# bentotten/radiation_ppo

Hardware: AMD Instinct MI355X
Metric: env steps/sec (whole node) at 4096 envs; PPO iters/sec at 1/2/4/8 GPUs (higher is better)
Workload: dtype f32 policy / f64+int32 env

## Files before the change

include/radsearch.h:

```cpp
#ifndef RADSEARCH_H
#define RADSEARCH_H

#include <stddef.h>
#include <stdint.h>

#ifdef __cplusplus
extern "C" {
#endif

#define RS_ABI_VERSION 4
#define RS_OBS_DIM 11
#define RS_NUM_ACTIONS 9
#define RS_MAX_AGENTS 8
#define RS_MAX_OBS 7

typedef void* rs_stream_t;
typedef struct rs_handle rs_handle;

enum {
    RS_OK = 0,
    RS_ERR_INVALID_ARG = 1,
    RS_ERR_HIP = 2,
    RS_ERR_WORKSPACE = 3,
    RS_ERR_UNSUPPORTED = 4
};

enum {
    RS_ENVERR_ZERO_DIST = 1,
    RS_ENVERR_IDLE_STALL = 2,
    RS_ENVERR_CORRECT_CAP = 4,
    RS_ENVERR_BAD_ACTION = 8,
    RS_ENVERR_NO_PATH = 16
};

typedef struct rs_config {
    int32_t num_envs;
    int32_t num_agents;
    int32_t obstruction_count;
    int32_t enforce_grid_boundaries;
    int32_t bbox[4];
    int32_t observation_area[2];
    int32_t falloff;
    int32_t geom_group_size;
    uint32_t seed;
    uint32_t env_id_base;
    int32_t coord_noise;
    int32_t debug_spawn;
} rs_config;

typedef struct rs_info {
    uint8_t* out_of_bounds;
    int32_t* out_of_bounds_count;
    uint8_t* blocked;
    uint8_t* collision;
} rs_info;

const char* rs_strerror(int code);
int rs_abi_version(void);

size_t rs_state_bytes(const rs_config* cfg);

int rs_create(const rs_config* cfg, void* workspace, size_t workspace_bytes, rs_stream_t stream, rs_handle** out);
void rs_destroy(rs_handle* h);

int rs_state_field(rs_handle* h, const char* name, void** dev_ptr, int32_t* elem_bytes, int32_t* rows, int32_t* cols);

int rs_set_epoch_end(rs_handle* h, rs_stream_t stream);

int rs_reset(rs_handle* h, const uint8_t* mask, float* obs, float* reward, float* team, uint8_t* done,
             const rs_info* info, rs_stream_t stream);

int rs_refresh(rs_handle* h, const uint8_t* mask, const int32_t* src_xy, const int32_t* det_xy, const int32_t* intensity,
               const int32_t* bkg, const int32_t* num_obs, const int32_t* rects, float* obs, float* reward, float* team,
               uint8_t* done, const rs_info* info, rs_stream_t stream);

int rs_step(rs_handle* h, const int8_t* actions, float* obs, float* reward, float* team, uint8_t* done,
            const rs_info* info, rs_stream_t stream);

int rs_action_uniforms(rs_handle* h, float* u, rs_stream_t stream);

int rs_error_flags(rs_handle* h, rs_stream_t stream, uint32_t* flags_out);

int rs_gae(const float* rew, const float* val, const uint8_t* cut, const float* last_val, float* adv, float* ret,
           int32_t T, int32_t M, double gamma, double lam, rs_stream_t stream);

typedef struct rs_mlp_params {
    const float *w1, *b1, *w2, *b2, *w3, *b3;
} rs_mlp_params;

int rs_policy_forward(const rs_mlp_params* actor, const rs_mlp_params* critic, const float* x, int32_t M,
                      float* logits, float* value, rs_stream_t stream);

typedef struct rs_rollout_args {
    int32_t steps_per_epoch;
    int32_t steps_per_episode;
    float* obs;
    int64_t* act;
    float* logp;
    float* val;
    float* rew;
    float* last_val;
    uint8_t* cut;
    float* source_tar;
    float* cur_obs;
    double* w_count;
    double* w_mean;
    double* w_sq;
    double* w_std;
    int32_t* steps_in_ep;
    float* ep_ret;
    int32_t* done_count;
    int32_t* oob_count;
    double* ep_ret_sum;
    double* ep_len_sum;
    int32_t* ep_count;
    double* ep_ret_sq_sum;
    float* ep_ret_max;
    float* ep_ret_min;
} rs_rollout_args;

int rs_rollout(rs_handle* h, const rs_mlp_params* actor, const rs_mlp_params* critic, const rs_rollout_args* args,
               rs_stream_t stream);

typedef struct rs_ppo_batch {
    const float* x;
    const int64_t* act;
    const float* adv;
    const float* ret;
    const float* logp_old;
    const float* w;
    int32_t M;
    float clip_ratio, alpha, vf_coef;
} rs_ppo_batch;

size_t rs_ppo_grad_workspace_bytes(void);
#define RS_PPO_STATS_TAIL 16
#define RS_PPO_GRAD_FLOATS (10441 + RS_PPO_STATS_TAIL)
int rs_ppo_grad(const rs_mlp_params* actor, const rs_mlp_params* critic, const rs_ppo_batch* batch, float* grads,
                double* stats, void* workspace, const int32_t* stop_flag, rs_stream_t stream);

typedef struct rs_update_state {
    int32_t adam_step;
    int32_t stopped;
    int32_t iters;
    int32_t pad;
    double last_stats[5];
} rs_update_state;

int rs_adam_step(const rs_mlp_params* actor, const rs_mlp_params* critic, const float* grads, float* m, float* v,
                 const double* stats, rs_update_state* state, float lr, float kl_threshold, rs_stream_t stream);

int rs_ppo_update_step(const rs_mlp_params* actor, const rs_mlp_params* critic, const rs_ppo_batch* batch, float* grads,
                       double* stats, void* workspace, float* m, float* v, rs_update_state* state, float lr, float kl_threshold,
                       rs_stream_t stream);

typedef struct rs_maps rs_maps;
size_t rs_maps_state_bytes(int32_t num_envs, int32_t num_agents, int32_t steps_per_episode, int32_t map_x, int32_t map_y);
int rs_maps_create(int32_t num_envs, int32_t num_agents, int32_t steps_per_episode, int32_t map_x, int32_t map_y,
                   double resolution_accuracy, const float* visit_table, void* workspace, size_t workspace_bytes,
                   rs_stream_t stream, rs_maps** out);
void rs_maps_destroy(rs_maps* m);
int rs_maps_reset(rs_maps* m, const uint8_t* mask, rs_stream_t stream);
int rs_maps_update(rs_maps* m, rs_handle* env, const float* obs, const float* pred, const uint8_t* mask, rs_stream_t stream);
int rs_maps_stack(rs_maps* m, float* actor_stack, float* critic_stack, rs_stream_t stream);
int rs_maps_field(rs_maps* m, const char* name, void** dev_ptr, int32_t* elem_bytes, int32_t* rows, int32_t* cols);

int32_t rs_cnn_trunk_slab_row(int32_t in_channels);
int32_t rs_cnn_trunk_slab_rows(int64_t num_samples, int32_t in_channels);
int32_t rs_cnn_trunk_scratch_floats(int32_t in_channels);
int rs_cnn_trunk_forward(const float* maps, const int64_t* cells, const int64_t* pcells, int32_t num_agents, int32_t agent,
                         int64_t num_samples, const float* w1, const float* b1, const float* w2, const float* b2, float* a2,
                         float* p1, uint8_t* amax, uint16_t* relu_mask, float* wscratch, rs_stream_t stream);
int rs_cnn_trunk_backward(const float* maps, const int64_t* cells, const int64_t* pcells, int32_t num_agents, int32_t agent,
                          int64_t num_samples, const float* w2, const float* da2, const uint16_t* relu_mask, const float* p1,
                          const uint8_t* amax, float* slab, float* wscratch, rs_stream_t stream);

#define RS_PFGRU_PARTICLES 40
#define RS_PFGRU_HIDDEN 24
#define RS_PFGRU_WEIGHT_FLOATS 3472
int rs_pfgru_step(const float* weights, const float* obs, float* h, float* p, const int64_t* base_key, const int64_t* episode,
                  const int64_t* calls, const uint8_t* mask, int32_t carry_hidden, double alpha, float* pred, int32_t num_envs,
                  int32_t num_agents, rs_stream_t stream);
int rs_pfgru_pass(const float* weights, const float* obs, float* h, float* p, const int64_t* base_key, const int64_t* episode,
                  const int64_t* calls, double alpha, float* pred, const int32_t* alive, int32_t steps, int32_t episodes, rs_stream_t stream);
int rs_pfgru_step_recorded(const float* weights, const float* obs, float* h, float* p, const float* eps, const int32_t* idx,
                           const uint8_t* mask, int32_t carry_hidden, double alpha, float* pred, int32_t num_envs, int32_t num_agents,
                           rs_stream_t stream);
int rs_pfgru_reset(float* h, float* p, const int64_t* base_key, const int64_t* episode, const int64_t* calls, const uint8_t* mask,
                   int32_t num_envs, int32_t num_agents, rs_stream_t stream);

int32_t rs_pfgru_sized_weight_floats(int32_t hidden);
int rs_pfgru_sized_step(const float* weights, const float* obs, float* h, float* p, const int64_t* base_key, const int64_t* episode,
                        const int64_t* calls, const uint8_t* mask, int32_t carry_hidden, double alpha, float* pred, int32_t num_envs,
                        int32_t num_agents, int32_t hidden, rs_stream_t stream);
int rs_pfgru_sized_pass(const float* weights, const float* obs, float* h, float* p, const int64_t* base_key, const int64_t* episode,
                        const int64_t* calls, double alpha, float* pred, const int32_t* alive, int32_t steps, int32_t episodes, int32_t hidden,
                        rs_stream_t stream);
int rs_pfgru_sized_step_recorded(const float* weights, const float* obs, float* h, float* p, const float* eps, const int32_t* idx,
                                 const uint8_t* mask, int32_t carry_hidden, double alpha, float* pred, int32_t num_envs, int32_t num_agents,
                                 int32_t hidden, rs_stream_t stream);
int rs_pfgru_sized_reset(float* h, float* p, const int64_t* base_key, const int64_t* episode, const int64_t* calls, const uint8_t* mask,
                         int32_t num_envs, int32_t num_agents, int32_t hidden, rs_stream_t stream);

int rs_pfgru_draws(const int64_t* keys, int32_t episodes, int32_t steps, float* h0, float* eps, double* u, rs_stream_t stream);

#define RS_PFGRU_TRAIN_WEIGHT_FLOATS 3680
#define RS_PFGRU_TRAIN_GRAD_FLOATS 3376
int rs_pfgru_train(const float* weights, const float* obs, const float* target, const float* bp, const int64_t* lens, const float* w_ep,
                   const float* h0, const float* eps, const double* u, float* hs, float* ps, float* gates, int32_t* idx, float* loss,
                   float* grads, int32_t steps, int32_t episodes, double alpha, double l2_weight, double l1_weight, double elbo_weight,
                   rs_stream_t stream);
int rs_pfgru_train_keyed(const float* weights, const float* obs, const float* target, const float* bp, const int64_t* lens, const float* w_ep,
                         const int64_t* keys, float* h0, float* hs, float* ps, float* gates, int32_t* idx, float* loss, float* grads, int32_t steps,
                         int32_t episodes, double alpha, double l2_weight, double l1_weight, double elbo_weight, rs_stream_t stream);

int32_t rs_pfgru_sized_train_weight_floats(int32_t hidden);
int32_t rs_pfgru_sized_train_grad_floats(int32_t hidden);
int rs_pfgru_sized_draws(const int64_t* keys, int32_t episodes, int32_t steps, int32_t hidden, float* h0, float* eps, double* u,
                         rs_stream_t stream);
int rs_pfgru_sized_train(const float* weights, const float* obs, const float* target, const float* bp, const int64_t* lens, const float* w_ep,
                         const float* h0, const float* eps, const double* u, float* hs, float* ps, float* gates, int32_t* idx, float* loss,
                         float* grads, int32_t steps, int32_t episodes, double alpha, double l2_weight, double l1_weight, double elbo_weight,
                         int32_t hidden, rs_stream_t stream);

#define RS_GRU_HIDDEN 24
int rs_gru_forward(const float* gi, const float* h0, const float* whh_t, const float* bhh, float* hs, float* gates, int32_t steps,
                   int32_t episodes, rs_stream_t stream);
int rs_gru_backward(const float* dhs, const float* hs, const float* gates, const float* h0, const float* whh, float* dgi, float* dgh,
                    int32_t steps, int32_t episodes, rs_stream_t stream);

#define RS_RNN_POLICY_WEIGHT_FLOATS 5296
int rs_rnn_policy_step(const float* weights, const float* x, const float* loc, const float* h, const float* u, float* h_out,
                       float* logits, float* value, int64_t* act, float* logp, int32_t num_envs, rs_stream_t stream);
int rs_rnn_policy_step_rows(const float* weights, const float* x, int32_t x_stride, const float* loc, int32_t loc_stride, const float* h,
                            const float* u, int32_t u_stride, float* h_out, float* value, int64_t* act, float* logp, int8_t* act8,
                            int32_t act8_stride, const uint8_t* mask, int32_t num_envs, rs_stream_t stream);

int rs_a2c_heads_loss(const float* weights, const float* hs, const int64_t* act, const float* adv, const float* ret, const float* logp_old,
                      const float* sample_weight, float* dhs, float* dfac, float* tfac, float* stats, int64_t samples, double clip_ratio,
                      double vf_coef, rs_stream_t stream);

int32_t rs_rnn_sized_weight_floats(int32_t hid, int32_t pol, int32_t val);
int32_t rs_gru_sized_weight_floats(int32_t hid);
int32_t rs_gru_sized_gate_floats(int32_t hid);
int rs_rnn_sized_step(const float* weights, int32_t hid, int32_t pol, int32_t val, const float* x, int32_t x_stride, const float* loc,
                      int32_t loc_stride, const float* h, const float* u, int32_t u_stride, float* h_out, float* logits, float* value,
                      int64_t* act, float* logp, int8_t* act8, int32_t act8_stride, const uint8_t* mask, int32_t num_envs, rs_stream_t stream);
int rs_gru_sized_forward(const float* gi, const float* h0, const float* weights, float* hs, float* gates, int32_t hid, int32_t steps,
                         int32_t episodes, rs_stream_t stream);
int rs_gru_sized_backward(const float* dhs, const float* hs, const float* gates, const float* h0, const float* weights, float* dgi, float* dgh,
                          int32_t hid, int32_t steps, int32_t episodes, rs_stream_t stream);
int rs_a2c_sized_heads_loss(const float* weights, int32_t hid, int32_t pol, int32_t val, const float* hs, const int64_t* act, const float* adv,
                            const float* ret, const float* logp_old, const float* sample_weight, float* dhs, float* dfac, float* tfac,
                            float* stats, int64_t samples, double clip_ratio, double vf_coef, rs_stream_t stream);
int rs_gru_h0_reset_sized(float* h, const int64_t* base_key, const int64_t* episodes_begun, const uint8_t* mask, double scale, int32_t hid,
                          int32_t num_envs, int32_t num_agents, rs_stream_t stream);

int rs_cnn_trunk_prepare(int32_t in_channels, const float* w1, const float* b1, const float* w2, const float* b2, float* wscratch,
                         rs_stream_t stream);
int rs_cnn_trunk_infer(const float* maps, const int64_t* cells, const int64_t* pcells, int32_t num_agents, int32_t agent, int64_t num_samples,
                       const float* wscratch, float* a2, rs_stream_t stream);

int32_t rs_cnn_sized_slab_row(int32_t in_channels);
int32_t rs_cnn_sized_slab_rows(int64_t num_samples, int32_t map_side, int32_t in_channels);
int rs_cnn_sized_forward(const float* maps, const int64_t* cells, const int64_t* pcells, int32_t num_agents, int32_t agent,
                         int64_t num_samples, int32_t map_side, const float* w1, const float* b1, const float* w2, const float* b2,
                         float* a2, float* p1, uint8_t* amax, uint16_t* relu_mask, rs_stream_t stream);
int rs_cnn_sized_infer(const float* maps, const int64_t* cells, const int64_t* pcells, int32_t num_agents, int32_t agent, int64_t num_samples,
                       int32_t map_side, const float* w1, const float* b1, const float* w2, const float* b2, float* a2, rs_stream_t stream);
int rs_cnn_sized_backward(const float* maps, const int64_t* cells, const int64_t* pcells, int32_t num_agents, int32_t agent,
                          int64_t num_samples, int32_t map_side, const float* w2, const float* da2, const uint16_t* relu_mask,
                          const float* p1, const uint8_t* amax, float* slab, int32_t slab_rows, rs_stream_t stream);

int rs_cnn_head(const float* y1, const float* w2, const float* b2, const float* w3, const float* b3, int32_t out_dim, const float* u,
                int32_t u_stride, int64_t* act, float* logp, int8_t* act8, int32_t act8_stride, float* value, int32_t value_copies,
                int64_t value_stride, const uint8_t* mask, int32_t num_envs, rs_stream_t stream);

int rs_actor_loss(const float* logits, const int64_t* act, const float* adv, const float* logp_old, const float* sample_weight,
                  float* dlogits, float* stats, int64_t samples, double clip_ratio, rs_stream_t stream);

int rs_gru_h0_reset(float* h, const int64_t* base_key, const int64_t* episodes_begun, const uint8_t* mask, double scale, int32_t num_envs,
                    int32_t num_agents, rs_stream_t stream);

int rs_welford_update(double* count, double* mean, double* sq, double* std, const float* reading, int64_t stride, const uint8_t* mask,
                      int32_t num_envs, int32_t num_agents, rs_stream_t stream);
int rs_welford_reset(double* count, double* mean, double* sq, double* std, const uint8_t* mask, int32_t num_envs, int32_t num_agents,
                     rs_stream_t stream);
int rs_welford_standardize(const double* mean, const double* std, const float* reading, int64_t stride, float* out, int64_t out_stride,
                           int32_t streams, rs_stream_t stream);

int rs_epoch_stats(const uint8_t* out_of_bounds, const uint8_t* done, const float* ep_ret, const int32_t* steps_in_ep, const uint8_t* over,
                   double* acc_oob, double* acc_done, double* ep_cnt, double* ep_len, double* ret_sum, double* ret_sq, double* ret_max,
                   double* ret_min, int32_t num_envs, int32_t num_agents, rs_stream_t stream);

int rs_store_rows(const int64_t* t, const int64_t* act, const float* logp_val_boot, const float* x, const int32_t* src_x, const int32_t* src_y,
                  const float* rew, const uint8_t* cut, const uint8_t* boot, int64_t* buf_act, float* buf_logp, float* buf_val,
                  float* buf_last_val, float* buf_obs, float* buf_source, float* buf_rew, uint8_t* buf_cut, int32_t num_envs,
                  int32_t num_agents, int32_t steps_per_epoch, rs_stream_t stream);

typedef struct {
    int32_t num_envs, num_agents, steps_per_episode, team_reward;
    const float* env_obs;
    const float* env_reward;
    const float* env_team;
    const uint8_t* env_done;
    float* obs;
    float* ep_ret;
    int32_t* steps_in_ep;
    double* w_count; double* w_mean; double* w_sq; double* w_std;
    float* x;
    float* xb;
    float* reward_used;
    uint8_t* over; uint8_t* cut; uint8_t* boot;
    int64_t* pf_episode; int64_t* pf_calls; int64_t* episodes_begun;
    int64_t* t;
    const uint8_t* env_oob;
    const int32_t* env_src_x; const int32_t* env_src_y;
    uint8_t* done_copy; uint8_t* oob_copy;
    int32_t* src_copy;
    int64_t* complete_len;
} rs_collect_state;
int rs_collect_pre(const rs_collect_state* c, rs_stream_t stream);
int rs_collect_post_step(const rs_collect_state* c, int32_t epoch_ended, rs_stream_t stream);
int rs_collect_post_reset(const rs_collect_state* c, int32_t reset_hidden, rs_stream_t stream);

#ifdef __cplusplus
}
#endif
#endif
```

radiation_ppo_amd/_lib.py:

```python
import ctypes as C
import os

import torch

_PKG = os.path.dirname(os.path.abspath(__file__))
LIB_PATH = os.environ.get("RS_LIB_PATH") or os.path.join(_PKG, "lib", "librs_hip.so")

RS_OBS_DIM = 11
RS_MAX_AGENTS = 8
RS_MAX_OBS = 7

ENVERR_ZERO_DIST = 1
ENVERR_IDLE_STALL = 2
ENVERR_CORRECT_CAP = 4
ENVERR_BAD_ACTION = 8
ENVERR_NO_PATH = 16


class RsConfig(C.Structure):
    _fields_ = [
        ("num_envs", C.c_int32), ("num_agents", C.c_int32), ("obstruction_count", C.c_int32),
        ("enforce_grid_boundaries", C.c_int32), ("bbox", C.c_int32 * 4), ("observation_area", C.c_int32 * 2),
        ("falloff", C.c_int32), ("geom_group_size", C.c_int32), ("seed", C.c_uint32), ("env_id_base", C.c_uint32),
        ("coord_noise", C.c_int32), ("debug_spawn", C.c_int32),
    ]


class RsCollectState(C.Structure):
    _fields_ = [("num_envs", C.c_int32), ("num_agents", C.c_int32), ("steps_per_episode", C.c_int32), ("team_reward", C.c_int32)] + [
        (n, C.c_void_p) for n in ("env_obs", "env_reward", "env_team", "env_done", "obs", "ep_ret", "steps_in_ep", "w_count", "w_mean", "w_sq",
                                  "w_std", "x", "xb", "reward_used", "over", "cut", "boot", "pf_episode", "pf_calls", "episodes_begun", "t",
                                  "env_oob", "env_src_x", "env_src_y", "done_copy", "oob_copy", "src_copy", "complete_len")]


class RsMlpParams(C.Structure):
    _fields_ = [(n, C.c_void_p) for n in ("w1", "b1", "w2", "b2", "w3", "b3")]


class RsRolloutArgs(C.Structure):
    _fields_ = [("steps_per_epoch", C.c_int32), ("steps_per_episode", C.c_int32)] + [
        (n, C.c_void_p) for n in ("obs", "act", "logp", "val", "rew", "last_val", "cut", "source_tar", "cur_obs", "w_count",
                                  "w_mean", "w_sq", "w_std", "steps_in_ep", "ep_ret", "done_count", "oob_count",
                                  "ep_ret_sum", "ep_len_sum", "ep_count", "ep_ret_sq_sum", "ep_ret_max", "ep_ret_min")]


class RsPpoBatch(C.Structure):
    _fields_ = [("x", C.c_void_p), ("act", C.c_void_p), ("adv", C.c_void_p), ("ret", C.c_void_p), ("logp_old", C.c_void_p),
                ("w", C.c_void_p), ("M", C.c_int32), ("clip_ratio", C.c_float), ("alpha", C.c_float), ("vf_coef", C.c_float)]


class RsInfo(C.Structure):
    _fields_ = [("out_of_bounds", C.c_void_p), ("out_of_bounds_count", C.c_void_p), ("blocked", C.c_void_p),
                ("collision", C.c_void_p)]


SYMBOLS = [
    ("rs_strerror", C.c_char_p, [C.c_int]),
    ("rs_abi_version", C.c_int, []),
    ("rs_state_bytes", C.c_size_t, [C.POINTER(RsConfig)]),
    ("rs_create", C.c_int, [C.POINTER(RsConfig), C.c_void_p, C.c_size_t, C.c_void_p, C.POINTER(C.c_void_p)]),
    ("rs_destroy", None, [C.c_void_p]),
    ("rs_state_field", C.c_int, [C.c_void_p, C.c_char_p, C.POINTER(C.c_void_p), C.POINTER(C.c_int32),
                                 C.POINTER(C.c_int32), C.POINTER(C.c_int32)]),
    ("rs_set_epoch_end", C.c_int, [C.c_void_p, C.c_void_p]),
    ("rs_reset", C.c_int, [C.c_void_p, C.c_void_p, C.c_void_p, C.c_void_p, C.c_void_p, C.c_void_p,
                           C.POINTER(RsInfo), C.c_void_p]),
    ("rs_refresh", C.c_int, [C.c_void_p, C.c_void_p, C.c_void_p, C.c_void_p, C.c_void_p, C.c_void_p, C.c_void_p, C.c_void_p,
                             C.c_void_p, C.c_void_p, C.c_void_p, C.c_void_p, C.POINTER(RsInfo), C.c_void_p]),
    ("rs_step", C.c_int, [C.c_void_p, C.c_void_p, C.c_void_p, C.c_void_p, C.c_void_p, C.c_void_p,
                          C.POINTER(RsInfo), C.c_void_p]),
    ("rs_action_uniforms", C.c_int, [C.c_void_p, C.c_void_p, C.c_void_p]),
    ("rs_error_flags", C.c_int, [C.c_void_p, C.c_void_p, C.POINTER(C.c_uint32)]),
    ("rs_policy_forward", C.c_int, [C.POINTER(RsMlpParams), C.POINTER(RsMlpParams), C.c_void_p, C.c_int32, C.c_void_p,
                                    C.c_void_p, C.c_void_p]),
    ("rs_rollout", C.c_int, [C.c_void_p, C.POINTER(RsMlpParams), C.POINTER(RsMlpParams), C.POINTER(RsRolloutArgs), C.c_void_p]),
    ("rs_ppo_grad_workspace_bytes", C.c_size_t, []),
    ("rs_ppo_grad", C.c_int, [C.POINTER(RsMlpParams), C.POINTER(RsMlpParams), C.POINTER(RsPpoBatch), C.c_void_p, C.c_void_p,
                              C.c_void_p, C.c_void_p, C.c_void_p]),
    ("rs_adam_step", C.c_int, [C.POINTER(RsMlpParams), C.POINTER(RsMlpParams), C.c_void_p, C.c_void_p, C.c_void_p, C.c_void_p,
                               C.c_void_p, C.c_float, C.c_float, C.c_void_p]),
    ("rs_ppo_update_step", C.c_int, [C.POINTER(RsMlpParams), C.POINTER(RsMlpParams), C.POINTER(RsPpoBatch), C.c_void_p, C.c_void_p,
                                     C.c_void_p, C.c_void_p, C.c_void_p, C.c_void_p, C.c_float, C.c_float, C.c_void_p]),
    ("rs_maps_state_bytes", C.c_size_t, [C.c_int32, C.c_int32, C.c_int32, C.c_int32, C.c_int32]),
    ("rs_maps_create", C.c_int, [C.c_int32, C.c_int32, C.c_int32, C.c_int32, C.c_int32, C.c_double, C.c_void_p, C.c_void_p,
                                 C.c_size_t, C.c_void_p, C.POINTER(C.c_void_p)]),
    ("rs_maps_destroy", None, [C.c_void_p]),
    ("rs_maps_reset", C.c_int, [C.c_void_p, C.c_void_p, C.c_void_p]),
    ("rs_maps_update", C.c_int, [C.c_void_p, C.c_void_p, C.c_void_p, C.c_void_p, C.c_void_p, C.c_void_p]),
    ("rs_maps_stack", C.c_int, [C.c_void_p, C.c_void_p, C.c_void_p, C.c_void_p]),
    ("rs_maps_field", C.c_int, [C.c_void_p, C.c_char_p, C.POINTER(C.c_void_p), C.POINTER(C.c_int32), C.POINTER(C.c_int32),
                                C.POINTER(C.c_int32)]),
    ("rs_cnn_trunk_slab_row", C.c_int32, [C.c_int32]),
    ("rs_cnn_trunk_slab_rows", C.c_int32, [C.c_int64, C.c_int32]),
    ("rs_cnn_trunk_scratch_floats", C.c_int32, [C.c_int32]),
    ("rs_cnn_trunk_forward", C.c_int, [C.c_void_p, C.c_void_p, C.c_void_p, C.c_int32, C.c_int32, C.c_int64, C.c_void_p, C.c_void_p,
                                       C.c_void_p, C.c_void_p, C.c_void_p, C.c_void_p, C.c_void_p, C.c_void_p, C.c_void_p, C.c_void_p]),
    ("rs_cnn_trunk_backward", C.c_int, [C.c_void_p, C.c_void_p, C.c_void_p, C.c_int32, C.c_int32, C.c_int64, C.c_void_p, C.c_void_p,
                                        C.c_void_p, C.c_void_p, C.c_void_p, C.c_void_p, C.c_void_p, C.c_void_p]),
    ("rs_gae", C.c_int, [C.c_void_p, C.c_void_p, C.c_void_p, C.c_void_p, C.c_void_p, C.c_void_p, C.c_int32,
                         C.c_int32, C.c_double, C.c_double, C.c_void_p]),
    ("rs_pfgru_step", C.c_int, [C.c_void_p, C.c_void_p, C.c_void_p, C.c_void_p, C.c_void_p, C.c_void_p, C.c_void_p, C.c_void_p,
                                C.c_int32, C.c_double, C.c_void_p, C.c_int32, C.c_int32, C.c_void_p]),
    ("rs_pfgru_step_recorded", C.c_int, [C.c_void_p] * 7 + [C.c_int32, C.c_double, C.c_void_p, C.c_int32, C.c_int32, C.c_void_p]),
    ("rs_pfgru_pass", C.c_int, [C.c_void_p] * 7 + [C.c_double, C.c_void_p, C.c_void_p, C.c_int32, C.c_int32, C.c_void_p]),
    ("rs_pfgru_reset", C.c_int, [C.c_void_p, C.c_void_p, C.c_void_p, C.c_void_p, C.c_void_p, C.c_void_p, C.c_int32, C.c_int32,
                                 C.c_void_p]),
    ("rs_pfgru_sized_weight_floats", C.c_int32, [C.c_int32]),
    ("rs_pfgru_sized_step", C.c_int, [C.c_void_p] * 8 + [C.c_int32, C.c_double, C.c_void_p, C.c_int32, C.c_int32, C.c_int32, C.c_void_p]),
    ("rs_pfgru_sized_pass", C.c_int, [C.c_void_p] * 7 + [C.c_double, C.c_void_p, C.c_void_p, C.c_int32, C.c_int32, C.c_int32, C.c_void_p]),
    ("rs_pfgru_sized_step_recorded", C.c_int, [C.c_void_p] * 7 + [C.c_int32, C.c_double, C.c_void_p, C.c_int32, C.c_int32, C.c_int32,
                                                                    C.c_void_p]),
    ("rs_pfgru_sized_reset", C.c_int, [C.c_void_p] * 6 + [C.c_int32, C.c_int32, C.c_int32, C.c_void_p]),
    ("rs_pfgru_draws", C.c_int, [C.c_void_p, C.c_int32, C.c_int32, C.c_void_p, C.c_void_p, C.c_void_p, C.c_void_p]),
    ("rs_pfgru_train", C.c_int, [C.c_void_p] * 15 + [C.c_int32, C.c_int32, C.c_double, C.c_double, C.c_double, C.c_double, C.c_void_p]),
    ("rs_pfgru_train_keyed", C.c_int, [C.c_void_p] * 14 + [C.c_int32, C.c_int32, C.c_double, C.c_double, C.c_double, C.c_double, C.c_void_p]),
    ("rs_pfgru_sized_train_weight_floats", C.c_int32, [C.c_int32]),
    ("rs_pfgru_sized_train_grad_floats", C.c_int32, [C.c_int32]),
    ("rs_pfgru_sized_draws", C.c_int, [C.c_void_p, C.c_int32, C.c_int32, C.c_int32, C.c_void_p, C.c_void_p, C.c_void_p, C.c_void_p]),
    ("rs_pfgru_sized_train", C.c_int, [C.c_void_p] * 15 + [C.c_int32, C.c_int32, C.c_double, C.c_double, C.c_double, C.c_double, C.c_int32,
                                       C.c_void_p]),
    ("rs_rnn_policy_step", C.c_int, [C.c_void_p] * 10 + [C.c_int32, C.c_void_p]),
    ("rs_rnn_policy_step_rows", C.c_int, [C.c_void_p, C.c_void_p, C.c_int32, C.c_void_p, C.c_int32, C.c_void_p, C.c_void_p, C.c_int32, C.c_void_p,
                                          C.c_void_p, C.c_void_p, C.c_void_p, C.c_void_p, C.c_int32, C.c_void_p, C.c_int32, C.c_void_p]),
    ("rs_collect_pre", C.c_int, [C.POINTER(RsCollectState), C.c_void_p]),
    ("rs_collect_post_step", C.c_int, [C.POINTER(RsCollectState), C.c_int32, C.c_void_p]),
    ("rs_collect_post_reset", C.c_int, [C.POINTER(RsCollectState), C.c_int32, C.c_void_p]),
    ("rs_welford_update", C.c_int, [C.c_void_p] * 5 + [C.c_int64, C.c_void_p, C.c_int32, C.c_int32, C.c_void_p]),
    ("rs_welford_reset", C.c_int, [C.c_void_p] * 5 + [C.c_int32, C.c_int32, C.c_void_p]),
    ("rs_welford_standardize", C.c_int, [C.c_void_p] * 3 + [C.c_int64, C.c_void_p, C.c_int64, C.c_int32, C.c_void_p]),
    ("rs_gru_h0_reset", C.c_int, [C.c_void_p] * 4 + [C.c_double, C.c_int32, C.c_int32, C.c_void_p]),
    ("rs_epoch_stats", C.c_int, [C.c_void_p] * 13 + [C.c_int32, C.c_int32, C.c_void_p]),
    ("rs_a2c_heads_loss", C.c_int, [C.c_void_p] * 11 + [C.c_int64, C.c_double, C.c_double, C.c_void_p]),
    ("rs_actor_loss", C.c_int, [C.c_void_p] * 7 + [C.c_int64, C.c_double, C.c_void_p]),
    ("rs_cnn_trunk_prepare", C.c_int, [C.c_int32] + [C.c_void_p] * 6),
    ("rs_cnn_trunk_infer", C.c_int, [C.c_void_p, C.c_void_p, C.c_void_p, C.c_int32, C.c_int32, C.c_int64, C.c_void_p, C.c_void_p, C.c_void_p]),
    ("rs_cnn_sized_slab_row", C.c_int32, [C.c_int32]),
    ("rs_cnn_sized_slab_rows", C.c_int32, [C.c_int64, C.c_int32, C.c_int32]),
    ("rs_cnn_sized_forward", C.c_int, [C.c_void_p, C.c_void_p, C.c_void_p, C.c_int32, C.c_int32, C.c_int64, C.c_int32] + [C.c_void_p] * 9),
    ("rs_cnn_sized_infer", C.c_int, [C.c_void_p, C.c_void_p, C.c_void_p, C.c_int32, C.c_int32, C.c_int64, C.c_int32] + [C.c_void_p] * 6),
    ("rs_cnn_sized_backward", C.c_int, [C.c_void_p, C.c_void_p, C.c_void_p, C.c_int32, C.c_int32, C.c_int64, C.c_int32] + [C.c_void_p] * 6
     + [C.c_int32, C.c_void_p]),
    ("rs_cnn_head", C.c_int, [C.c_void_p] * 5 + [C.c_int32, C.c_void_p, C.c_int32, C.c_void_p, C.c_void_p, C.c_void_p, C.c_int32, C.c_void_p,
                              C.c_int32, C.c_int64, C.c_void_p, C.c_int32, C.c_void_p]),
    ("rs_store_rows", C.c_int, [C.c_void_p] * 17 + [C.c_int32, C.c_int32, C.c_int32, C.c_void_p]),
    ("rs_gru_forward", C.c_int, [C.c_void_p, C.c_void_p, C.c_void_p, C.c_void_p, C.c_void_p, C.c_void_p, C.c_int32, C.c_int32, C.c_void_p]),
    ("rs_gru_backward", C.c_int, [C.c_void_p, C.c_void_p, C.c_void_p, C.c_void_p, C.c_void_p, C.c_void_p, C.c_void_p, C.c_int32,
                                  C.c_int32, C.c_void_p]),
    ("rs_rnn_sized_weight_floats", C.c_int32, [C.c_int32, C.c_int32, C.c_int32]),
    ("rs_gru_sized_weight_floats", C.c_int32, [C.c_int32]),
    ("rs_gru_sized_gate_floats", C.c_int32, [C.c_int32]),
    ("rs_rnn_sized_step", C.c_int, [C.c_void_p, C.c_int32, C.c_int32, C.c_int32, C.c_void_p, C.c_int32, C.c_void_p, C.c_int32, C.c_void_p,
                                    C.c_void_p, C.c_int32] + [C.c_void_p] * 6 + [C.c_int32, C.c_void_p, C.c_int32, C.c_void_p]),
    ("rs_gru_sized_forward", C.c_int, [C.c_void_p] * 5 + [C.c_int32, C.c_int32, C.c_int32, C.c_void_p]),
    ("rs_gru_sized_backward", C.c_int, [C.c_void_p] * 7 + [C.c_int32, C.c_int32, C.c_int32, C.c_void_p]),
    ("rs_a2c_sized_heads_loss", C.c_int, [C.c_void_p, C.c_int32, C.c_int32, C.c_int32] + [C.c_void_p] * 10
     + [C.c_int64, C.c_double, C.c_double, C.c_void_p]),
    ("rs_gru_h0_reset_sized", C.c_int, [C.c_void_p] * 4 + [C.c_double, C.c_int32, C.c_int32, C.c_int32, C.c_void_p]),
]

_lib = None

EVENTS = None


class timed:
    def __init__(self, name: str):
        self.name = name

    def __enter__(self):
        self.ev = None
        if EVENTS is not None and not torch.cuda.is_current_stream_capturing():
            self.ev = (torch.cuda.Event(enable_timing=True), torch.cuda.Event(enable_timing=True))
            self.ev[0].record()
        return self

    def __exit__(self, *exc):
        if self.ev is not None:
            self.ev[1].record()
            EVENTS.setdefault(self.name, []).append(self.ev)
        return False


def load():
    global _lib
    if _lib is not None:
        return _lib
    if not os.path.exists(LIB_PATH):
        raise RuntimeError(
            f"{LIB_PATH} is missing: the MI355X HIP extension has not been built "
            "(run `python -c 'import __graft_entry__ as g; g.build()'` or `python radiation_ppo_amd/build.py`). "
            "There is no CPU fallback.")
    lib = C.CDLL(LIB_PATH)
    for name, restype, argtypes in SYMBOLS:
        fn = getattr(lib, name)
        fn.restype = restype
        fn.argtypes = argtypes
    if lib.rs_abi_version() != 4:
        raise RuntimeError("librs_hip.so ABI version mismatch")
    _lib = lib
    return lib


def check(code: int, what: str = "") -> None:
    if code != 0:
        msg = load().rs_strerror(code).decode()
        raise RuntimeError(f"librs_hip {what}: {msg} (code {code})")
```

radiation_ppo_amd/build.py:

```python
import os
import shutil
import subprocess
import sys
from concurrent.futures import ThreadPoolExecutor

PKG = os.path.dirname(os.path.abspath(__file__))
ROOT = os.path.dirname(PKG)
CSRC = os.path.join(PKG, "csrc")
LIBDIR = os.path.join(PKG, "lib")
OBJDIR = os.path.join(LIBDIR, "obj")
LIB = os.path.join(LIBDIR, "librs_hip.so")

SOURCES = ["rs_env.hip", "rs_ppo.hip", "rs_maps.hip", "rs_cnn.hip", "rs_cnn_sized.hip", "rs_pfgru.hip", "rs_gru.hip", "rs_pfgru_train.hip", "rs_rnn_policy.hip", "rs_welford.hip", "rs_cnn_loss.hip",
           "rs_rnn_sized.hip", "rs_pfgru_sized.hip", "rs_pfgru_sized_train.hip"]
CFLAGS = ["--offload-arch=gfx950", "-O3", "-std=c++17", "-fPIC", "-ffp-contract=off", "-fno-fast-math", "-Wall",
          "-Wno-unused-function"]
EXTRA_CFLAGS = {"rs_ppo.hip": ["-fno-slp-vectorize"], "rs_rnn_sized.hip": ["-mllvm", "-pragma-unroll-threshold=1000000"],
                "rs_pfgru_sized.hip": ["-mllvm", "-pragma-unroll-threshold=1000000"]}


def hipcc() -> str:
    for c in (os.environ.get("HIPCC"), shutil.which("hipcc"), "/opt/rocm/bin/hipcc"):
        if c and os.path.exists(c):
            return c
    raise RuntimeError("hipcc not found: the MI355X extension cannot be built")


def _deps():
    return [os.path.join(CSRC, f) for f in os.listdir(CSRC)] + [os.path.join(ROOT, "include", "radsearch.h"), __file__]


def _newer(target: str, deps) -> bool:
    if not os.path.exists(target):
        return True
    t = os.path.getmtime(target)
    return any(os.path.getmtime(d) > t for d in deps)


def build(force: bool = False, verbose: bool = True, defines=(), suffix: str = "") -> str:
    deps = _deps()
    lib = LIB.replace(".so", suffix + ".so")
    if not force and not _newer(lib, deps):
        return lib
    os.makedirs(OBJDIR, exist_ok=True)
    cc = hipcc()

    def compile_one(src):
        obj = os.path.join(OBJDIR, src.replace(".hip", suffix + ".o"))
        if force or _newer(obj, deps):
            cmd = [cc] + CFLAGS + EXTRA_CFLAGS.get(src, []) + ["-D" + d for d in defines] + ["-c", os.path.join(CSRC, src), "-o", obj]
            if verbose:
                print("[radiation_ppo_amd.build]", " ".join(cmd), flush=True)
            subprocess.run(cmd, check=True)
        return obj

    try:
        cpus = len(os.sched_getaffinity(0))
    except AttributeError:
        cpus = os.cpu_count() or 1
    jobs = max(1, min(len(SOURCES), cpus, int(os.environ.get("MAX_JOBS") or cpus)))
    order = sorted(SOURCES, key=lambda f: f not in ("rs_rnn_sized.hip", "rs_pfgru_sized.hip"))
    with ThreadPoolExecutor(max_workers=jobs) as ex:
        done = dict(zip(order, ex.map(compile_one, order)))
    objs = [done[f] for f in SOURCES]
    cmd = [cc, "--offload-arch=gfx950", "-shared", "-fPIC"] + objs + ["-o", lib]
    if verbose:
        print("[radiation_ppo_amd.build]", " ".join(cmd), flush=True)
    subprocess.run(cmd, check=True)
    return lib


if __name__ == "__main__":
    if "--stamps" in sys.argv:
        build(force="--force" in sys.argv, defines=["RS_K7_STAMPS"], suffix="_stamps")
    else:
        build(force="--force" in sys.argv)
```

radiation_ppo_amd/ppo.py:

```python
import ctypes as C
import os
from dataclasses import dataclass
from typing import Any, Dict, List, Optional

import torch
import torch.distributed as dist
import torch.nn as nn

from . import _lib
from .envs import RadSearchVec, gae as rs_gae_call


class FFActorCritic(nn.Module):

    def __init__(self, state_dim: int = 11, action_dim: int = 8, hidden: int = 64):
        super().__init__()
        self.actor = nn.Sequential(nn.Linear(state_dim, hidden), nn.Tanh(), nn.Linear(hidden, hidden), nn.Tanh(),
                                   nn.Linear(hidden, action_dim), nn.Softmax(dim=-1))
        self.critic = nn.Sequential(nn.Linear(state_dim, hidden), nn.Tanh(), nn.Linear(hidden, hidden), nn.Tanh(),
                                    nn.Linear(hidden, 1))

    def logits(self, x: torch.Tensor) -> torch.Tensor:
        for layer in list(self.actor)[:-1]:
            x = layer(x)
# ... 398 lines not shown

    def _update_agent_fused(self, X, act, adv, ret, logp_old, w) -> UpdateResult:
        if self._fused is None:
            self._fused = FusedPPOGrad(self.agent)
        f = self._fused
        lr = self.actor_learning_rate * (0.99 ** (self.epochs_done // 100))
        thr = 1.5 * self.target_kl
        f.begin_update()
        one_rank = _world() == 1 and not os.environ.get("RS_PPO_SPLIT_TAIL")
        for _ in range(self.train_pi_iters):
            if one_rank:
                f.step(X, act, adv, ret, logp_old, w, self.clip_ratio, self.alpha, lr=lr, kl_threshold=thr)
                continue
            stats, grads = f(X, act, adv, ret, logp_old, w, self.clip_ratio, self.alpha, use_stop_flag=True)
            if _world() > 1:
                f.allreduce()
            f.adam_step(lr, thr)
        kk, stopped, _, last = f.read_state()
        self.epochs_done += 1
        return UpdateResult(stop_iteration=kk, loss_policy=last[4], loss_critic=last[3], loss_predictor=0.0,
                            kl_divergence=last[0], Entropy=last[1], ClipFrac=last[2], LocLoss=0.0)

    def save(self, path: str) -> None:
        torch.save(self.agent.state_dict(), path)

    def load(self, path: str) -> None:
        self.agent.load_state_dict(torch.load(path, map_location=self.device, weights_only=True))

    def resume_state(self) -> Dict[str, Any]:
        st: Dict[str, Any] = dict(model=self.agent.state_dict(), epochs_done=self.epochs_done,
                                  pi_optimizer=self.pi_optimizer.state_dict(), pi_scheduler=self.pi_scheduler.state_dict())
        if self._fused is not None:
            f = self._fused
            st["fused"] = dict(m=f.m.clone(), v=f.v.clone(), adam_step=int(f.state_i32[0].item()))
        return st

    def load_resume_state(self, st: Dict[str, Any]) -> None:
        self.agent.load_state_dict(st["model"])
        self.epochs_done = int(st["epochs_done"])
        self.pi_optimizer.load_state_dict(st["pi_optimizer"])
        self.pi_scheduler.load_state_dict(st["pi_scheduler"])
        if "fused" in st:
            if self._fused is None:
                self._fused = FusedPPOGrad(self.agent)
            f = self._fused
            f.m.copy_(st["fused"]["m"]); f.v.copy_(st["fused"]["v"])
            f.state_i32[0] = int(st["fused"]["adam_step"])


def normalize_advantages(adv: torch.Tensor) -> torch.Tensor:
    n = torch.tensor([adv.numel()], dtype=torch.float64, device=adv.device)
    s = adv.double().sum().view(1)
    if _world() > 1:
        pack = torch.cat([s, n])
        Collectives.all_reduce_sum(pack)
        s, n = pack[0:1], pack[1:2]
    mean = (s / n).float()
    sq = ((adv - mean) ** 2).double().sum().view(1)
    if _world() > 1:
        Collectives.all_reduce_sum(sq)
    std = torch.sqrt(sq / n).float()
    return (adv - mean) / std


class EpochStats:

    def __init__(self, A: int, device):
        f64 = dict(dtype=torch.float64, device=device)
        self.oob = torch.zeros(A, **f64)
        self.done = torch.zeros(A, **f64)
        self.ep_cnt = torch.zeros((), **f64)
        self.ep_len = torch.zeros((), **f64)
        self.ret_sum = torch.zeros(A, **f64)
        self.ret_sq = torch.zeros(A, **f64)
        self.ret_max = torch.full((A,), float("-inf"), **f64)
        self.ret_min = torch.full((A,), float("inf"), **f64)

    def zero_(self) -> None:
        for t in (self.oob, self.done, self.ep_cnt, self.ep_len, self.ret_sum, self.ret_sq):
            t.zero_()
        self.ret_max.fill_(float("-inf")); self.ret_min.fill_(float("inf"))

    def step(self, out_of_bounds: torch.Tensor, done: torch.Tensor) -> None:
        self.oob += out_of_bounds.double().sum(dim=0)
        self.done += done.double().sum(dim=0)

    def episodes(self, ep_ret: torch.Tensor, steps_in_ep: torch.Tensor, over: torch.Tensor) -> None:
        m = over.unsqueeze(1)
        r = ep_ret.double()
        self.ret_sum += (r * m).sum(dim=0)
        self.ret_sq += (r * r * m).sum(dim=0)
        self.ret_max.copy_(torch.maximum(self.ret_max, torch.where(m, r, torch.full_like(r, float("-inf"))).max(dim=0).values))
        self.ret_min.copy_(torch.minimum(self.ret_min, torch.where(m, r, torch.full_like(r, float("inf"))).min(dim=0).values))
        self.ep_len += (steps_in_ep.double() * over).sum()
        self.ep_cnt += over.double().sum()

    def step_and_episodes(self, out_of_bounds: torch.Tensor, done: torch.Tensor, ep_ret: torch.Tensor, steps_in_ep: torch.Tensor,
                          over: torch.Tensor) -> None:
        ok = (self.oob.is_cuda and out_of_bounds.dtype == torch.uint8 and done.dtype == torch.uint8 and ep_ret.dtype == torch.float32
              and steps_in_ep.dtype == torch.int32 and over.dtype == torch.bool
              and all(t.is_contiguous() for t in (out_of_bounds, done, ep_ret, steps_in_ep, over)))
        if not ok:
            self.step(out_of_bounds, done)
            self.episodes(ep_ret, steps_in_ep, over)
            return
        N, A = ep_ret.shape
        _lib.check(_lib.load().rs_epoch_stats(out_of_bounds.data_ptr(), done.data_ptr(), ep_ret.data_ptr(), steps_in_ep.data_ptr(),
                                              over.view(torch.uint8).data_ptr(), self.oob.data_ptr(), self.done.data_ptr(),
                                              self.ep_cnt.data_ptr(), self.ep_len.data_ptr(), self.ret_sum.data_ptr(), self.ret_sq.data_ptr(),
                                              self.ret_max.data_ptr(), self.ret_min.data_ptr(), N, A,
                                              C.c_void_p(torch.cuda.current_stream(self.oob.device).cuda_stream)), "rs_epoch_stats")

    def result(self) -> Dict[str, torch.Tensor]:
        return dict(DoneCount=self.done.clone(), OutOfBound=self.oob.clone(), EpCount=self.ep_cnt.clone(), EpLenSum=self.ep_len.clone(),
                    EpRetSum=self.ret_sum.clone(), EpRetSqSum=self.ret_sq.clone(), EpRetMax=self.ret_max.clone(), EpRetMin=self.ret_min.clone())


def _welford_state(w: "DeviceWelford"):
    return dict(count=w.count.clone(), mean=w.mean.clone(), sq=w.sq.clone(), std=w.std.clone())


def _welford_load(w: "DeviceWelford", st) -> None:
    w.count.copy_(st["count"]); w.mean.copy_(st["mean"]); w.sq.copy_(st["sq"]); w.std.copy_(st["std"])


class Collector:

    def __init__(self, env: RadSearchVec, agents: Dict[int, VecAgentPPO], steps_per_epoch: int, steps_per_episode: int,
                 global_critic_flag: bool = False, standardize: bool = True):
        self.env, self.agents = env, agents
        self.T, self.L = steps_per_epoch, steps_per_episode
        self.N, self.A = env.num_envs, env.number_agents
        self.team_reward = global_critic_flag
        self.standardize = standardize
        dev = env.device
        self.buf = RolloutBuffer(self.T, self.N, self.A, _lib.RS_OBS_DIM, dev)
        self.stat = DeviceWelford((self.N, self.A), dev)
        self.steps_in_ep = torch.zeros(self.N, dtype=torch.int32, device=dev)
        self.ep_ret = torch.zeros(self.N, self.A, dtype=torch.float32, device=dev)
        self._u = torch.empty(self.N, self.A, dtype=torch.float32, device=dev)
        self._act8 = torch.empty(self.N, self.A, dtype=torch.int8, device=dev)
        self.stats: Dict[str, torch.Tensor] = {}
        self.obs = None
        self.started = False

    def _x(self, obs: torch.Tensor) -> torch.Tensor:
        if not self.standardize:
            return obs
        x = obs.clone()
        self.stat.standardize(obs[..., 0], out=x[..., 0])
        return x

    def start(self) -> None:
        obs, *_ = self.env.reset()
        self.obs = obs.clone()
        self.stat.update(self.obs[..., 0])
        self.started = True

    @torch.no_grad()
    def collect(self) -> Dict[str, torch.Tensor]:
        if not self.started:
            self.start()
        env, buf, T, L, N, A = self.env, self.buf, self.T, self.L, self.N, self.A
        dev = env.device
        acc = EpochStats(A, dev)
        for t in range(T):
            x = self._x(self.obs)
            env.action_uniforms(self._u)
            for a, ag in self.agents.items():
                act, logp, v = ag.agent.act(x[:, a], self._u[:, a])
                buf.act[t, :, a] = act
                buf.logp[t, :, a] = logp
                buf.val[t, :, a] = v
                self._act8[:, a] = act.to(torch.int8)
            buf.obs[t] = x
            buf.source_tar[t, :, 0] = env.state("src_x")[0].float()
            buf.source_tar[t, :, 1] = env.state("src_y")[0].float()
            next_obs, rew, team, done, info = env.step(self._act8)
            r_used = team.unsqueeze(1).expand(N, A) if self.team_reward else rew
            buf.rew[t] = r_used
            self.ep_ret += r_used
            self.steps_in_ep += 1
            terminal = done.bool().any(dim=1)
            acc.step(info["out_of_bounds"], done)
            timeout = self.steps_in_ep == L
            episode_over = terminal | timeout
            epoch_ended = t == T - 1
            cut = episode_over | epoch_ended
            buf.cut[t] = cut.unsqueeze(1).to(torch.uint8).expand(N, A)
            self.stat.update(next_obs[..., 0])
            self.obs = next_obs.clone()
            boot = timeout | epoch_ended
            xb = self._x(self.obs)
            for a, ag in self.agents.items():
                vb = ag.agent.critic(xb[:, a]).squeeze(-1)
                buf.last_val[t, :, a] = torch.where((boot & cut).bool(), vb, torch.zeros_like(vb))
            acc.episodes(self.ep_ret, self.steps_in_ep, episode_over)
            if epoch_ended:
                env.set_epoch_end()
            self.stat.reset(cut)
            obs_r, *_ = env.reset(cut)
            self.obs = obs_r.clone()
            self.ep_ret = torch.where(cut.unsqueeze(1), torch.zeros_like(self.ep_ret), self.ep_ret)
            self.steps_in_ep = torch.where(cut, torch.zeros_like(self.steps_in_ep), self.steps_in_ep)
            self.stat.update(self.obs[..., 0], mask=cut)
        buf.finish(self.agents[0].gamma, self.agents[0].lam)
        return acc.result()

    def update(self) -> Dict[int, UpdateResult]:
        return ppo_update_from_buffer(self)

    def resume_state(self) -> Dict[str, Any]:
        if not self.started:
            self.start()
        return dict(env=self.env.snapshot(), stat=_welford_state(self.stat), steps_in_ep=self.steps_in_ep.clone(),
                    ep_ret=self.ep_ret.clone(), obs=self.obs.clone())

    def load_resume_state(self, st: Dict[str, Any]) -> None:
        if not self.started:
            self.start()
        self.env.restore(st["env"])
        _welford_load(self.stat, st["stat"])
        self.steps_in_ep, self.ep_ret, self.obs = st["steps_in_ep"].clone(), st["ep_ret"].clone(), st["obs"].clone()


class FusedCollector:

    def __init__(self, env: RadSearchVec, agents: Dict[int, VecAgentPPO], steps_per_epoch: int, steps_per_episode: int,
                 global_critic_flag: bool = False, standardize: bool = True):
        assert env.number_agents == 1 and len(agents) == 1 and env.num_envs % 16 == 0 and standardize
        assert not global_critic_flag
        self.env, self.agents = env, agents
        self.T, self.L, self.N, self.A = steps_per_epoch, steps_per_episode, env.num_envs, 1
        dev = env.device
        self.buf = RolloutBuffer(self.T, self.N, 1, _lib.RS_OBS_DIM, dev)
        N = self.N
        f64 = dict(dtype=torch.float64, device=dev)
        self.cur_obs = torch.zeros(N, _lib.RS_OBS_DIM, dtype=torch.float32, device=dev)
        self.w_count, self.w_mean, self.w_sq = (torch.zeros(N, **f64) for _ in range(3))
        self.w_std = torch.ones(N, **f64)
        self.steps_in_ep = torch.zeros(N, dtype=torch.int32, device=dev)
        self.ep_ret = torch.zeros(N, dtype=torch.float32, device=dev)
        self.done_count = torch.zeros(N, dtype=torch.int32, device=dev)
        self.oob_count = torch.zeros(N, dtype=torch.int32, device=dev)
        self.ep_count = torch.zeros(N, dtype=torch.int32, device=dev)
        self.ep_ret_sum = torch.zeros(N, **f64)
        self.ep_len_sum = torch.zeros(N, **f64)
        self.ep_ret_sq = torch.zeros(N, **f64)
        self.ep_ret_max = torch.zeros(N, dtype=torch.float32, device=dev)
        self.ep_ret_min = torch.zeros(N, dtype=torch.float32, device=dev)
        b = self.buf
        self._args = _lib.RsRolloutArgs(
            self.T, self.L, b.obs.data_ptr(), b.act.data_ptr(), b.logp.data_ptr(), b.val.data_ptr(), b.rew.data_ptr(),
            b.last_val.data_ptr(), b.cut.data_ptr(), b.source_tar.data_ptr(), self.cur_obs.data_ptr(),
            self.w_count.data_ptr(), self.w_mean.data_ptr(), self.w_sq.data_ptr(), self.w_std.data_ptr(),
            self.steps_in_ep.data_ptr(), self.ep_ret.data_ptr(), self.done_count.data_ptr(), self.oob_count.data_ptr(),
            self.ep_ret_sum.data_ptr(), self.ep_len_sum.data_ptr(), self.ep_count.data_ptr(),
            self.ep_ret_sq.data_ptr(), self.ep_ret_max.data_ptr(), self.ep_ret_min.data_ptr())
        self.started = False

    def start(self) -> None:
        obs, *_ = self.env.reset()
        self.cur_obs.copy_(obs[:, 0])
        st = DeviceWelford((self.N,), self.env.device)
        st.update(self.cur_obs[:, 0])
        self.w_count.copy_(st.count); self.w_mean.copy_(st.mean); self.w_sq.copy_(st.sq); self.w_std.copy_(st.std)
        self.started = True

    @torch.no_grad()
    def collect(self) -> Dict[str, torch.Tensor]:
        import ctypes as C
        if not self.started:
            self.start()
        ac = self.agents[0].agent
        pa, pc = mlp_params(ac.actor), mlp_params(ac.critic)
        with _lib.timed("rs_rollout"):
            _lib.check(self.env.lib.rs_rollout(self.env._h, C.byref(pa), C.byref(pc), C.byref(self._args), self.env._stream()),
                       "rs_rollout")
        with _lib.timed("rs_gae"):
            self.buf.finish(self.agents[0].gamma, self.agents[0].lam)
        one = lambda t: t.double().sum().view(1)
        return dict(DoneCount=one(self.done_count), OutOfBound=one(self.oob_count), EpCount=self.ep_count.double().sum(),
                    EpLenSum=self.ep_len_sum.sum(), EpRetSum=one(self.ep_ret_sum), EpRetSqSum=one(self.ep_ret_sq),
                    EpRetMax=self.ep_ret_max.double().max().view(1), EpRetMin=self.ep_ret_min.double().min().view(1))

    def update(self) -> Dict[int, UpdateResult]:
        return ppo_update_from_buffer(self)

    _RESUME = ("cur_obs", "w_count", "w_mean", "w_sq", "w_std", "steps_in_ep", "ep_ret")

    def resume_state(self) -> Dict[str, Any]:
        if not self.started:
            self.start()
        return dict(env=self.env.snapshot(), **{k: getattr(self, k).clone() for k in self._RESUME})

    def load_resume_state(self, st: Dict[str, Any]) -> None:
        if not self.started:
            self.start()
        self.env.restore(st["env"])
        for k in self._RESUME:
            getattr(self, k).copy_(st[k])


def ppo_update_from_buffer(col) -> Dict[int, UpdateResult]:
    buf = col.buf
    n_total = col.N * _world()
    w = (buf.episode_weights() / n_total).reshape(-1)
    out = {}
    for a, ag in col.agents.items():
        adv = normalize_advantages(buf.adv[:, :, a]).reshape(-1)
        X = buf.obs[:, :, a].reshape(-1, buf.obs.shape[-1])
        out[a] = ag.update_agent(X, buf.act[:, :, a].reshape(-1), adv, buf.ret[:, :, a].reshape(-1),
                                 buf.logp[:, :, a].reshape(-1), w)
    return out
```

Before: 39.69 million.

## Add fused HIP kernel for episode weights and advantage normalization in PPO update

Adds a HIP routine that computes per-step episode weights from cut flags and normalizes advantages with double-precision mean and std reductions. It runs as three kernels in place of several PyTorch ops, and it is used by default on a single GPU. The goal is to cut launch count and host overhead in the PPO update preparation. The cost is a separate code path whose numerics must match the torch version, and it recomputes the weights once per agent.

```diff
diff --git a/include/radsearch.h b/include/radsearch.h
--- a/include/radsearch.h
+++ b/include/radsearch.h
@@ -83,6 +83,10 @@
 
 int rs_gae(const float* rew, const float* val, const uint8_t* cut, const float* last_val, float* adv, float* ret,
            int32_t T, int32_t M, double gamma, double lam, rs_stream_t stream);
+
+size_t rs_ppo_prepare_workspace_bytes(int32_t N);
+int rs_ppo_prepare(const uint8_t* cut, const float* adv, int32_t T, int32_t N, float inv_n_total, void* workspace, float* w, float* adv_norm,
+                   rs_stream_t stream);
 
 typedef struct rs_mlp_params {
     const float *w1, *b1, *w2, *b2, *w3, *b3;
diff --git a/radiation_ppo_amd/_lib.py b/radiation_ppo_amd/_lib.py
--- a/radiation_ppo_amd/_lib.py
+++ b/radiation_ppo_amd/_lib.py
@@ -81,6 +81,8 @@
                                C.c_void_p, C.c_float, C.c_float, C.c_void_p]),
     ("rs_ppo_update_step", C.c_int, [C.POINTER(RsMlpParams), C.POINTER(RsMlpParams), C.POINTER(RsPpoBatch), C.c_void_p, C.c_void_p,
                                      C.c_void_p, C.c_void_p, C.c_void_p, C.c_void_p, C.c_float, C.c_float, C.c_void_p]),
+    ("rs_ppo_prepare_workspace_bytes", C.c_size_t, [C.c_int32]),
+    ("rs_ppo_prepare", C.c_int, [C.c_void_p, C.c_void_p, C.c_int32, C.c_int32, C.c_float, C.c_void_p, C.c_void_p, C.c_void_p, C.c_void_p]),
     ("rs_maps_state_bytes", C.c_size_t, [C.c_int32, C.c_int32, C.c_int32, C.c_int32, C.c_int32]),
     ("rs_maps_create", C.c_int, [C.c_int32, C.c_int32, C.c_int32, C.c_int32, C.c_int32, C.c_double, C.c_void_p, C.c_void_p,
                                  C.c_size_t, C.c_void_p, C.POINTER(C.c_void_p)]),
diff --git a/radiation_ppo_amd/build.py b/radiation_ppo_amd/build.py
--- a/radiation_ppo_amd/build.py
+++ b/radiation_ppo_amd/build.py
@@ -12,7 +12,7 @@
 LIB = os.path.join(LIBDIR, "librs_hip.so")
 
 SOURCES = ["rs_env.hip", "rs_ppo.hip", "rs_maps.hip", "rs_cnn.hip", "rs_cnn_sized.hip", "rs_pfgru.hip", "rs_gru.hip", "rs_pfgru_train.hip", "rs_rnn_policy.hip", "rs_welford.hip", "rs_cnn_loss.hip",
-           "rs_rnn_sized.hip", "rs_pfgru_sized.hip", "rs_pfgru_sized_train.hip"]
+           "rs_rnn_sized.hip", "rs_pfgru_sized.hip", "rs_pfgru_sized_train.hip", "rs_ppo_prepare.hip"]
 CFLAGS = ["--offload-arch=gfx950", "-O3", "-std=c++17", "-fPIC", "-ffp-contract=off", "-fno-fast-math", "-Wall",
           "-Wno-unused-function"]
 EXTRA_CFLAGS = {"rs_ppo.hip": ["-fno-slp-vectorize"], "rs_rnn_sized.hip": ["-mllvm", "-pragma-unroll-threshold=1000000"],
diff --git a/radiation_ppo_amd/csrc/rs_ppo_prepare.hip b/radiation_ppo_amd/csrc/rs_ppo_prepare.hip
--- /dev/null
+++ b/radiation_ppo_amd/csrc/rs_ppo_prepare.hip
@@ -0,0 +1,143 @@
+#include <hip/hip_runtime.h>
+#include <stdint.h>
+
+#include "../../include/radsearch.h"
+
+#define RS_PREP_BLOCKS 256
+#define RS_PREP_THREADS 256
+#define RS_PREP_UNROLL 32
+
+namespace {
+
+struct RsPrepWs { double *col, *sq, *out; };
+
+__host__ __device__ inline RsPrepWs rs_prep_ws(void* workspace, int N) {
+    RsPrepWs w;
+    w.col = static_cast<double*>(workspace);
+    w.sq = w.col + N;
+    w.out = w.sq + RS_PREP_BLOCKS;
+    return w;
+}
+
+__global__ void __launch_bounds__(64) rs_prepare_columns_kernel(const uint8_t* __restrict__ cut, const float* __restrict__ adv, int T, int N,
+                                                                float inv_n_total, float* w, double* __restrict__ colsum) {
+    const int n = blockIdx.x * 64 + threadIdx.x;
+    if (n >= N) return;
+    float* wpos = w;
+    int pos = 0, closed = 0;
+    double s = 0.0;
+    int t = 0;
+    for (; t + RS_PREP_UNROLL <= T; t += RS_PREP_UNROLL) {
+        uint8_t c[RS_PREP_UNROLL];
+        float a[RS_PREP_UNROLL];
+#pragma unroll
+        for (int u = 0; u < RS_PREP_UNROLL; ++u) {
+            c[u] = cut[(size_t)(t + u) * N + n];
+            a[u] = adv[(size_t)(t + u) * N + n];
+        }
+#pragma unroll
+        for (int u = 0; u < RS_PREP_UNROLL; ++u) {
+            s += (double)a[u];
+            wpos[(size_t)(t + u) * N + n] = (float)pos;
+            const bool close = c[u] != 0;
+            closed += (close && t + u < T - 1) ? 1 : 0;
+            pos = close ? 0 : pos + 1;
+        }
+    }
+    for (; t < T; ++t) {
+        s += (double)adv[(size_t)t * N + n];
+        wpos[(size_t)t * N + n] = (float)pos;
+        const bool close = cut[(size_t)t * N + n] != 0;
+        closed += (close && t < T - 1) ? 1 : 0;
+        pos = close ? 0 : pos + 1;
+    }
+    colsum[n] = s;
+    const float n_ep = (float)(closed + 1);
+    int len = 0;
+    t = T - 1;
+    for (; t - RS_PREP_UNROLL + 1 >= 0; t -= RS_PREP_UNROLL) {
+        uint8_t c[RS_PREP_UNROLL];
+        float p[RS_PREP_UNROLL];
+#pragma unroll
+        for (int u = 0; u < RS_PREP_UNROLL; ++u) {
+            c[u] = cut[(size_t)(t - u) * N + n];
+            p[u] = wpos[(size_t)(t - u) * N + n];
+        }
+#pragma unroll
+        for (int u = 0; u < RS_PREP_UNROLL; ++u) {
+            if (t - u == T - 1 || c[u] != 0) len = (int)p[u] + 1;
+            w[(size_t)(t - u) * N + n] = (1.0f / (n_ep * (float)len)) * inv_n_total;
+        }
+    }
+    for (; t >= 0; --t) {
+        const float p = wpos[(size_t)t * N + n];
+        if (t == T - 1 || cut[(size_t)t * N + n] != 0) len = (int)p + 1;
+        w[(size_t)t * N + n] = (1.0f / (n_ep * (float)len)) * inv_n_total;
+    }
+}
+
+__device__ __forceinline__ double rs_prep_block_sum(double v, double* red) {
+    red[threadIdx.x] = v;
+    __syncthreads();
+    for (int k = RS_PREP_THREADS / 2; k > 0; k >>= 1) {
+        if ((int)threadIdx.x < k) red[threadIdx.x] += red[threadIdx.x + k];
+        __syncthreads();
+    }
+    const double r = red[0];
+    __syncthreads();
+    return r;
+}
+
+__global__ void __launch_bounds__(RS_PREP_THREADS) rs_prepare_sq_kernel(const float* __restrict__ adv, int M, int N, const double* __restrict__ colsum,
+                                                                         double* __restrict__ sqpart, double* __restrict__ out) {
+    __shared__ double red[RS_PREP_THREADS];
+    double s = 0.0;
+    for (int j = threadIdx.x; j < N; j += RS_PREP_THREADS) s += colsum[j];
+    s = rs_prep_block_sum(s, red);
+    const float mean = (float)(s / (double)M);
+    double q = 0.0;
+    for (int i = blockIdx.x * RS_PREP_THREADS + threadIdx.x; i < M; i += RS_PREP_BLOCKS * RS_PREP_THREADS) {
+        const float d = adv[i] - mean;
+        q += (double)(d * d);
+    }
+    q = rs_prep_block_sum(q, red);
+    if (threadIdx.x == 0) {
+        sqpart[blockIdx.x] = q;
+        if (blockIdx.x == 0) { out[0] = s; out[1] = (double)mean; }
+    }
+}
+
+__global__ void __launch_bounds__(RS_PREP_THREADS) rs_prepare_apply_kernel(const float* __restrict__ adv, int M, const double* __restrict__ sqpart,
+                                                                            double* __restrict__ out, float* __restrict__ adv_norm) {
+    __shared__ double red[RS_PREP_THREADS];
+    static_assert(RS_PREP_BLOCKS == RS_PREP_THREADS, "one partial sum per thread");
+    const double sq = rs_prep_block_sum(sqpart[threadIdx.x], red);
+    const float mean = (float)out[1];
+    const float sd = (float)sqrt(sq / (double)M);
+    if (blockIdx.x == 0 && threadIdx.x == 0) { out[2] = sq; out[3] = (double)sd; }
+    for (int i = blockIdx.x * RS_PREP_THREADS + threadIdx.x; i < M; i += gridDim.x * RS_PREP_THREADS) adv_norm[i] = (adv[i] - mean) / sd;
+}
+
+}
+
+extern "C" {
+
+size_t rs_ppo_prepare_workspace_bytes(int32_t N) {
+    return N < 1 ? 0 : sizeof(double) * ((size_t)N + RS_PREP_BLOCKS + 4);
+}
+
+int rs_ppo_prepare(const uint8_t* cut, const float* adv, int32_t T, int32_t N, float inv_n_total, void* workspace, float* w, float* adv_norm,
+                   rs_stream_t stream) {
+    if (!cut || !adv || !workspace || !w || !adv_norm || T < 1 || N < 1 || (int64_t)T * N > INT32_MAX) return RS_ERR_INVALID_ARG;
+    if (reinterpret_cast<uintptr_t>(workspace) & 7u) return RS_ERR_WORKSPACE;
+    hipStream_t s = static_cast<hipStream_t>(stream);
+    const RsPrepWs ws = rs_prep_ws(workspace, N);
+    const int M = T * N;
+    hipLaunchKernelGGL(rs_prepare_columns_kernel, dim3((N + 63) / 64), dim3(64), 0, s, cut, adv, T, N, inv_n_total, w, ws.col);
+    hipLaunchKernelGGL(rs_prepare_sq_kernel, dim3(RS_PREP_BLOCKS), dim3(RS_PREP_THREADS), 0, s, adv, M, N, ws.col, ws.sq, ws.out);
+    const int blocks = (M + 4 * RS_PREP_THREADS - 1) / (4 * RS_PREP_THREADS);
+    hipLaunchKernelGGL(rs_prepare_apply_kernel, dim3(blocks < 1024 ? blocks : 1024), dim3(RS_PREP_THREADS), 0, s, adv, M, ws.sq, ws.out, adv_norm);
+    return hipGetLastError() == hipSuccess ? RS_OK : RS_ERR_HIP;
+}
+
+}
diff --git a/radiation_ppo_amd/ppo.py b/radiation_ppo_amd/ppo.py
--- a/radiation_ppo_amd/ppo.py
+++ b/radiation_ppo_amd/ppo.py
@@ -724,13 +724,41 @@
             getattr(self, k).copy_(st[k])
 
 
+def ppo_prepare(cut: torch.Tensor, adv: torch.Tensor, n_total: int, ws: Optional[torch.Tensor] = None):
+    assert cut.dtype == torch.uint8 and adv.dtype == torch.float32 and cut.shape == adv.shape and adv.dim() == 2 and adv.is_cuda
+    cut, adv = cut.contiguous(), adv.contiguous()
+    T, N = adv.shape
+    lib = _lib.load()
+    if ws is None:
+        ws = prepare_workspace(N, adv.device)
+    w, adv_norm = torch.empty_like(adv), torch.empty_like(adv)
+    inv = (torch.tensor(1.0, dtype=torch.float32) / torch.tensor(float(n_total), dtype=torch.float32)).item()
+    with _lib.timed("rs_ppo_prepare"):
+        _lib.check(lib.rs_ppo_prepare(cut.data_ptr(), adv.data_ptr(), T, N, inv, ws.data_ptr(), w.data_ptr(), adv_norm.data_ptr(),
+                                      torch.cuda.current_stream(adv.device).cuda_stream), "rs_ppo_prepare")
+    return w, adv_norm
+
+
+def prepare_workspace(N: int, device) -> torch.Tensor:
+    return torch.empty(_lib.load().rs_ppo_prepare_workspace_bytes(N) // 8, dtype=torch.float64, device=device)
+
+
 def ppo_update_from_buffer(col) -> Dict[int, UpdateResult]:
     buf = col.buf
     n_total = col.N * _world()
-    w = (buf.episode_weights() / n_total).reshape(-1)
+    hip = _world() == 1 and buf.adv.is_cuda and not os.environ.get("RS_PPO_TORCH_PREPARE")
+    if hip:
+        if getattr(col, "_prep_ws", None) is None:
+            col._prep_ws = prepare_workspace(buf.N, buf.adv.device)
+    else:
+        w = (buf.episode_weights() / n_total).reshape(-1)
     out = {}
     for a, ag in col.agents.items():
-        adv = normalize_advantages(buf.adv[:, :, a]).reshape(-1)
+        if hip:
+            w2, adv2 = ppo_prepare(buf.cut[:, :, 0], buf.adv[:, :, a], n_total, col._prep_ws)
+            w, adv = w2.reshape(-1), adv2.reshape(-1)
+        else:
+            adv = normalize_advantages(buf.adv[:, :, a]).reshape(-1)
         X = buf.obs[:, :, a].reshape(-1, buf.obs.shape[-1])
         out[a] = ag.update_agent(X, buf.act[:, :, a].reshape(-1), adv, buf.ret[:, :, a].reshape(-1),
                                  buf.logp[:, :, a].reshape(-1), w)
```

Result: no change. 39.78 million (median of 4 runs) (+0.2%).
